# guanjq/targetdiff

Hardware: NVIDIA H100
Metric: molecules/sec (1000-step sampling, CrossDocked pocket shape) (higher is better)
Workload: dtype f32 (storage, LayerNorm, softmax, accumulation); GEMM operands as 2-piece bf16 splits on wgmma (3 products, ~16-bit operand mantissa)

## Files before the change

### targetdiff_b200/csrc/edge_mlp_v4.cu

```cuda
#include <stdio.h>
#include <stdlib.h>
#include <string.h>

#include "tdiff_common.cuh"
#include "hopper_mma.cuh"

namespace v4 {

constexpr int kTile = 64;
constexpr int kTabClassBytes = 2 * 128 * 128;
constexpr int kSrcStride = 512 + 32, kDst = 8;
constexpr int sSrc = 0, sDstRows = sSrc + kTile * kSrcStride, sMeta = sDstRows + kDst * 512, kStage = sMeta + kTile * 16;
constexpr int kMAtom = 32 * 128, kMPiece = 2 * kMAtom, kMImg = 2 * kMPiece;
template <int NOUT, bool FOLD>
struct Map {
  static constexpr int kCons = (NOUT == 128 && !FOLD) ? 3 : 2;
  static constexpr int kThreads = (kCons + 1) * 128;
  static constexpr int kProdRegs = kCons == 3 ? 32 : 40, kConsRegs = kCons == 3 ? 160 : 232;
  static constexpr int W = 0, T = W + 4 * 128 * 128, Par = T + kTabClassBytes, X = Par + 2 * 128 * 4,
                       M = X + kCons * 4 * 2 * 128 * 4, C = M + (FOLD ? kCons * kMImg : 0), Stage = C + (FOLD ? kCons * 32 * 4 : 0),
                       Bar = Stage + kCons * kStage, Smem = Bar + 8 * (1 + 2 * kCons);
  static constexpr bool kOrdered = kCons == 2;
  static constexpr int kPairBar = 1, kOrderBar = kPairBar + 2 * kCons, kFoldBar = kOrderBar + kCons;
  static_assert(M % 1024 == 0 && Stage % 128 == 0 && kStage % 128 == 0 && Smem <= 227 * 1024, "shared-memory map");
  static_assert(128 * kProdRegs + kCons * 128 * kConsRegs == kThreads * (65536 / kThreads / 8 * 8), "register split");
  static_assert(kFoldBar + kCons <= 16, "named barriers");
};

__device__ __forceinline__ uint32_t smem_u32(const void* p) { return (uint32_t)__cvta_generic_to_shared(p); }
__device__ __forceinline__ void mbar_init(uint32_t bar, uint32_t count) {
  asm volatile("mbarrier.init.shared::cta.b64 [%0], %1;" ::"r"(bar), "r"(count) : "memory");
}
__device__ __forceinline__ void mbar_wait(uint32_t bar, uint32_t parity) {
  asm volatile(
      "{\n\t.reg .pred p;\n\tWAIT_LOOP:\n\tmbarrier.try_wait.parity.shared::cta.b64 p, [%0], %1;\n\t@p bra WAIT_DONE;\n\tbra WAIT_LOOP;\n\t"
      "WAIT_DONE:\n\t}" ::"r"(bar), "r"(parity) : "memory");
}
__device__ __forceinline__ void mbar_expect_tx(uint32_t bar, uint32_t bytes) {
  asm volatile("mbarrier.arrive.expect_tx.shared::cta.b64 _, [%0], %1;" ::"r"(bar), "r"(bytes) : "memory");
}
__device__ __forceinline__ void bulk_g2s(uint32_t smem_dst, const void* gsrc, uint32_t bytes, uint32_t bar) {
  asm volatile("cp.async.bulk.shared::cluster.global.mbarrier::complete_tx::bytes [%0], [%1], %2, [%3];" ::"r"(smem_dst), "l"(gsrc), "r"(bytes),
               "r"(bar) : "memory");
}
__device__ __forceinline__ void fence_barrier_init() { asm volatile("fence.mbarrier_init.release.cluster;" ::: "memory"); }
__device__ __forceinline__ void mbar_arrive(uint32_t bar) { asm volatile("mbarrier.arrive.shared::cta.b64 _, [%0];" ::"r"(bar) : "memory"); }
__device__ __forceinline__ void mbar_expect_tx_only(uint32_t bar, uint32_t bytes) {
  asm volatile("mbarrier.expect_tx.shared::cta.b64 [%0], %1;" ::"r"(bar), "r"(bytes) : "memory");
}
__device__ __forceinline__ void named_bar_sync(int id, int nthreads) { asm volatile("bar.sync %0, %1;" ::"r"(id), "r"(nthreads) : "memory"); }
__device__ __forceinline__ void named_bar_arrive(int id, int nthreads) { asm volatile("bar.arrive %0, %1;" ::"r"(id), "r"(nthreads) : "memory"); }
template <int N> __device__ __forceinline__ void setmaxnreg_inc() { asm volatile("setmaxnreg.inc.sync.aligned.u32 %0;" ::"n"(N)); }
template <int N> __device__ __forceinline__ void setmaxnreg_dec() { asm volatile("setmaxnreg.dec.sync.aligned.u32 %0;" ::"n"(N)); }

__device__ __forceinline__ uint32_t cvt_bf16x2(float hi, float lo) {
  uint32_t d;
  asm("cvt.rn.bf16x2.f32 %0, %1, %2;" : "=r"(d) : "f"(hi), "f"(lo));
  return d;
}
__device__ __forceinline__ float ex2_approx(float x) { float y; asm("ex2.approx.ftz.f32 %0, %1;" : "=f"(y) : "f"(x)); return y; }
__device__ __forceinline__ void stg64(float* p, float a, float b) { asm volatile("st.global.v2.f32 [%0], {%1,%2};" ::"l"(p), "f"(a), "f"(b) : "memory"); }
__device__ __forceinline__ void stg128(float* p, float a, float b, float c, float d) {
  asm volatile("st.global.v4.f32 [%0], {%1,%2,%3,%4};" ::"l"(p), "f"(a), "f"(b), "f"(c), "f"(d) : "memory");
}

struct LnParams { float b[128]; float b2[128]; float mu[20]; };
struct AggArgs {
  const float* logits;
  const float* e_w;
  float* h;
  int key_softmax;
};

template <int N, int M, int LO_BIT>
__device__ __forceinline__ void transpose_reduce(float (&t)[N], int lane) {
  if constexpr (N > M) {
    constexpr int h = (N / M / 2) << LO_BIT;
    const bool up = lane & h;
#pragma unroll
    for (int i = 0; i < N / 2; ++i) {
      const float send = up ? t[i] : t[i + N / 2];
      const float keep = up ? t[i + N / 2] : t[i];
      t[i] = keep + __shfl_xor_sync(0xffffffffu, send, h);
    }
    transpose_reduce<N / 2, M, LO_BIT>(reinterpret_cast<float(&)[N / 2]>(t), lane);
  }
}
__device__ __forceinline__ void split2(float y0, float y1, uint32_t& hi, uint32_t& lo) {
  hi = cvt_bf16x2(y1, y0);
  const float r0 = __fsub_rn(y0, __uint_as_float(hi << 16)), r1 = __fsub_rn(y1, __uint_as_float(hi & 0xffff0000u));
  lo = cvt_bf16x2(r1, r0);
}

}

using namespace v4;

template <int NOUT, bool FOLD>
__global__ void __launch_bounds__(Map<NOUT, FOLD>::kThreads, 1)
edge_mlp_v4_kernel(const float* __restrict__ P, int zero_row, const int* __restrict__ src, const unsigned char* __restrict__ etype,
                   const float* __restrict__ dist_arr, const int* __restrict__ row_nodes, long long n_dst, long long split_dst,
                   const int* __restrict__ d_counts, int k, int offA, int offB, const unsigned char* __restrict__ w2_image,
                   const unsigned char* __restrict__ tab_image, float coeff, const float* __restrict__ qnode, float* __restrict__ out, int out_by_slot, AggArgs agg,
                   int cls, const __grid_constant__ LnParams lp) {
  static_assert(!FOLD || NOUT == 128, "the fold applies to the key MLPs");
  using L = Map<NOUT, FOLD>;
  constexpr int kCons = L::kCons, kThreads = L::kThreads;
  extern __shared__ __align__(1024) unsigned char smem_raw[];
  const uint32_t sbase = smem_u32(smem_raw);
  const uint32_t sW = sbase + L::W, sT = sbase + L::T, sBar = sbase + L::Bar;
  float* const s_b = reinterpret_cast<float*>(smem_raw + L::Par);
  float* const s_b2 = s_b + 128;
  const int tid = threadIdx.x, lane = tid & 31, warp = __shfl_sync(0xffffffffu, tid >> 5, 0);
  const int w = warp & 3, q = lane & 3;
  const int kshift = (k & (k - 1)) == 0 ? __ffs(k) - 1 : -1;
  auto row_dst = [&](long long idx, int& j) -> unsigned {
    const unsigned a = kshift >= 0 ? (unsigned)idx >> kshift : (unsigned)idx / (unsigned)k;
    j = (int)((unsigned)idx - a * (unsigned)k);
    return a;
  };

  if ((sbase & 1023u) != 0) __trap();
  if (d_counts) { n_dst = d_counts[0]; split_dst = d_counts[1]; }
  const long long n_rows = n_dst * k, split_rows = split_dst * k;
  const long long row_lo = cls ? split_rows : 0, row_hi = cls ? n_rows : split_rows;
  const long long n_tiles = row_hi > row_lo ? (row_hi - row_lo + kTile - 1) / kTile : 0;
  const long long my_tiles = (n_tiles > blockIdx.x) ? (n_tiles - blockIdx.x + gridDim.x - 1) / gridDim.x : 0;
  auto full_bar = [&](int c) { return sBar + 8u * (1 + c); };
  auto empty_bar = [&](int c) { return sBar + 8u * (1 + kCons + c); };

  constexpr int kWAtom = NOUT * 128;
  constexpr int kWPiece = 2 * kWAtom;
  constexpr uint32_t kWBytes = FOLD ? 4u * 128 * 128 : 2u * kWPiece;
  if (tid == 0) {
    mbar_init(sBar, 1);
    for (int c = 0; c < kCons; ++c) { mbar_init(full_bar(c), 32); mbar_init(empty_bar(c), 128); }
    fence_barrier_init();
    mbar_expect_tx(sBar, kWBytes + kTabClassBytes);
    bulk_g2s(sW, w2_image, kWBytes, sBar);
    bulk_g2s(sT, tab_image + (size_t)cls * kTabClassBytes, kTabClassBytes, sBar);
  }
  for (int i = tid; i < 128; i += kThreads) { s_b[i] = lp.b[i]; s_b2[i] = lp.b2[i]; }
  __syncthreads();

  if (warp < 4) {
    setmaxnreg_dec<L::kProdRegs>();
    if (warp >= kCons) return;
    const int c = warp;
    const uint32_t st = sbase + L::Stage + (uint32_t)c * kStage;
    for (long long it = c, use = 0; it < my_tiles; it += kCons, ++use) {
      const long long tile = blockIdx.x + it * (long long)gridDim.x, row0 = row_lo + tile * kTile;
      int j0;
      const unsigned a0 = row_dst(row0, j0);
      const long long last = (row0 + kTile - 1 < row_hi ? row0 + kTile - 1 : row_hi - 1);
      const int n_d = min(kDst, (int)(row_dst(last, j0) - a0) + 1);
      int s[2];
      int4 meta[2];
#pragma unroll
      for (int h = 0; h < 2; ++h) {
        const long long idx = row0 + lane + 32 * h;
        int jj = 0, ty = 3, slot = 0, node = -1;
        float dist = 0.f;
        s[h] = -1;
        if (idx < n_rows) {
          const unsigned a = row_dst(idx, jj);
          slot = a - a0 < (unsigned)kDst ? (int)(a - a0) + 1 : 0;
          node = row_nodes[a];
          if (node >= 0) {
            const size_t e = (size_t)node * k + jj;
            s[h] = src[e]; ty = etype[e]; dist = dist_arr[e];
          }
        }
        meta[h] = make_int4(node, s[h], __float_as_int(dist), ty | (slot << 8) | (jj << 16));
      }
      int dnode = -1;
      if (lane < n_d) dnode = row_nodes[a0 + lane];
      mbar_wait(empty_bar(c), (uint32_t)(use & 1) ^ 1u);
#pragma unroll
      for (int h = 0; h < 2; ++h) *reinterpret_cast<int4*>(smem_raw + L::Stage + c * kStage + sMeta + 16 * (lane + 32 * h)) = meta[h];
      if (lane == 0) mbar_expect_tx_only(full_bar(c), (uint32_t)(kTile + (FOLD ? 2 : 1) * n_d) * 512u);
      __syncwarp();
#pragma unroll
      for (int h = 0; h < 2; ++h)
        bulk_g2s(st + sSrc + (uint32_t)(lane + 32 * h) * kSrcStride, P + (size_t)(s[h] >= 0 ? s[h] : zero_row) * TD_NPROJ + offB, 512u, full_bar(c));
      if (lane < n_d) bulk_g2s(st + sDstRows + (uint32_t)lane * 512u, P + (size_t)(dnode >= 0 ? dnode : zero_row) * TD_NPROJ + offA, 512u, full_bar(c));
      if (FOLD && lane < n_d) bulk_g2s(st + sDstRows + (uint32_t)(2 + lane) * 512u, qnode + (size_t)(dnode >= 0 ? dnode : 0) * TD_H, 512u, full_bar(c));
      mbar_arrive(full_bar(c));
    }
    return;
  }

  setmaxnreg_inc<L::kConsRegs>();
  const int cwg = (warp >> 2) - 1;
  float mu[5];
#pragma unroll
  for (int m = 0; m < 5; ++m) mu[m] = lp.mu[5 * q + m];
  const float coeff2 = coeff * 1.4426950408889634f;
  mbar_wait(sBar, 0);

  const int r_base = 16 * w + (lane >> 2);
  const int pair_bar = L::kPairBar + 2 * cwg + (w >> 1);
  float* const xslot = reinterpret_cast<float*>(smem_raw + L::X) + (size_t)(cwg * 4 + w) * 256;
  float* const xpart = xslot + ((w & 1) ? -256 : 256);
  const bool do_agg = !FOLD && NOUT == 128 && qnode == nullptr && agg.logits != nullptr;
  const bool key_sm = NOUT == 128 && qnode != nullptr && agg.key_softmax;
  const unsigned char* const stage = smem_raw + L::Stage + cwg * kStage;
  const int ct = tid & 127, fu = ct & 7, fg = ct >> 3;
  const int fhd = 8 * (fg & 1) + 4 * (fu >> 2) + (fu & 3), fs = fu >> 2, frun = (fg >> 1) ^ (((fu >> 1) & 1) << 2);
  const int fn0 = 16 * ((fhd >> 1) & 1) + 2 * (fhd >> 2) + (fhd & 1);
  unsigned char* const mimg = smem_raw + L::M + cwg * kMImg;
  float* const s_c = reinterpret_cast<float*>(smem_raw + L::C) + cwg * 32;
  const int srow = k == 32 ? (w >> 1) : 0;
  const int order_mine = L::kOrderBar + cwg, order_next = L::kOrderBar + (cwg + 1) % kCons;
  auto order_wait = [&] { if constexpr (L::kOrdered) named_bar_sync(order_mine, 256); };
  auto order_pass = [&] { if constexpr (L::kOrdered) named_bar_arrive(order_next, 256); };
  const long long n_iter = (my_tiles + kCons - 1) / kCons;
  if (n_iter == 0) return;
  if (cwg == kCons - 1) order_pass();
  int set = 0;

  for (long long n = 0; n < n_iter; ++n, set ^= 1) {
    const long long it = n * kCons + cwg;
    if (it >= my_tiles) {
      if constexpr (L::kOrdered)
        for (int phase = 0; phase < 2; ++phase) { order_wait(); order_pass(); }
      continue;
    }
    const long long row0 = row_lo + (blockIdx.x + it * (long long)gridDim.x) * kTile;
    long long idx[2];
    int node[2], s[2], ty[2], jj[2], dsl[2];
    float dist[2];
    mbar_wait(full_bar(cwg), (uint32_t)(n & 1));
#pragma unroll
    for (int h = 0; h < 2; ++h) {
      idx[h] = row0 + r_base + 8 * h;
      const int4 m4 = *reinterpret_cast<const int4*>(stage + sMeta + 16 * (r_base + 8 * h));
      node[h] = m4.x; s[h] = m4.y; dist[h] = __int_as_float(m4.z);
      ty[h] = m4.w & 0xff; dsl[h] = ((m4.w >> 8) & 0xff) - 1; jj[h] = m4.w >> 16;
    }
    float ewp[2] = {0.f, 0.f};
    float4 qf[2][2];
    if constexpr (FOLD) {
#pragma unroll
      for (int h = 0; h < 2; ++h)
        if (key_sm && idx[h] < n_rows && node[h] >= 0) ewp[h] = agg.e_w[(size_t)node[h] * k + jj[h]];
#pragma unroll
      for (int sl = 0; sl < 2; ++sl)
#pragma unroll
        for (int hf = 0; hf < 2; ++hf) {
          float4 v = make_float4(0.f, 0.f, 0.f, 0.f);
          if (sl == 0 || k == 32) {
            v = *reinterpret_cast<const float4*>(stage + sDstRows + (2 + sl) * 512 + 32 * fhd + 16 * (hf ^ fs));
            v.x *= 0.35355339059327373f; v.y *= 0.35355339059327373f; v.z *= 0.35355339059327373f; v.w *= 0.35355339059327373f;
          }
          qf[sl][hf] = v;
        }
    }
    uint32_t ghi[4][4], glo[4][4];
#pragma unroll
    for (int h = 0; h < 2; ++h) {
      const bool ok = s[h] >= 0;
      float v[8];
#pragma unroll
      for (int m = 0; m < 5; ++m) {
        const float t = dist[h] - mu[m];
        v[m] = ok ? ex2_approx(coeff2 * (t * t)) : 0.0f;
      }
      v[5] = (ok && q == 3) ? 1.0f : 0.0f;
      v[6] = v[7] = 0.0f;
      const int half = ty[h] < 2 ? 1 : 0;
#pragma unroll
      for (int kk = 0; kk < 4; ++kk)
#pragma unroll
        for (int hk = 0; hk < 2; ++hk) {
          uint32_t hi, lo;
          split2(v[4 * (kk & 1) + 2 * hk], v[4 * (kk & 1) + 2 * hk + 1], hi, lo);
          const bool own = (kk >> 1) == half;
          ghi[kk][h + 2 * hk] = own ? hi : 0u;
          glo[kk][h + 2 * hk] = own ? lo : 0u;
        }
    }
    float x[64];
#pragma unroll
    for (int h = 0; h < 2; ++h) {
      const bool valid = s[h] >= 0;
      const float* ps = reinterpret_cast<const float*>(stage + sSrc + (r_base + 8 * h) * kSrcStride) + 2 * q;
      const float* pd = (dsl[h] >= 0 ? reinterpret_cast<const float*>(stage + sDstRows + dsl[h] * 512)
                                     : P + (size_t)(valid ? node[h] : zero_row) * TD_NPROJ + offA) + 2 * q;
#pragma unroll
      for (int i = 0; i < 16; ++i) {
        const float2 b = *reinterpret_cast<const float2*>(ps + 8 * i);
        float2 a = make_float2(0.f, 0.f);
        if (valid) a = *reinterpret_cast<const float2*>(pd + 8 * i);
        x[4 * i + 2 * h] = __fadd_rn(b.x, a.x);
        x[4 * i + 2 * h + 1] = __fadd_rn(b.y, a.y);
      }
    }
    mbar_arrive(empty_bar(cwg));
    wgmma_fence();
    order_wait();
#pragma unroll
    for (int term = 0; term < 3; ++term) {
#pragma unroll
      for (int kk = 0; kk < 4; ++kk)
        wgmma_n128_rs(x, term == 2 ? glo[kk] : ghi[kk], gmma_desc_sw128(sT + (term == 1 ? kTabClassBytes / 2 : 0) + kk * 32),
                      1u);
    }
    wgmma_commit();
    order_pass();
    if constexpr (FOLD) {
      const float* const w2s = reinterpret_cast<const float*>(smem_raw + L::W) + 8 * fhd;
#pragma unroll
      for (int jr = 0; jr < 2; ++jr) {
        const int f0 = 64 * jr + 8 * frun;
        float mv[2][8];
#pragma unroll
        for (int jf = 0; jf < 8; ++jf) {
          const float4 wa = *reinterpret_cast<const float4*>(w2s + (f0 + jf) * 128 + 4 * fs);
          const float4 wb = *reinterpret_cast<const float4*>(w2s + (f0 + jf) * 128 + 4 * (fs ^ 1));
#pragma unroll
          for (int sl = 0; sl < 2; ++sl) {
            const float4 qa = qf[sl][0], qb = qf[sl][1];
            const float pa = __fmaf_rn(wa.w, qa.w, __fmaf_rn(wa.z, qa.z, __fmaf_rn(wa.y, qa.y, wa.x * qa.x)));
            const float pb = __fmaf_rn(wb.w, qb.w, __fmaf_rn(wb.z, qb.z, __fmaf_rn(wb.y, qb.y, wb.x * qb.x)));
            mv[sl][jf] = pa + pb;
          }
        }
#pragma unroll
        for (int sl = 0; sl < 2; ++sl) {
          uint4 hi, lo;
          split2(mv[sl][0], mv[sl][1], hi.x, lo.x);
          split2(mv[sl][2], mv[sl][3], hi.y, lo.y);
          split2(mv[sl][4], mv[sl][5], hi.z, lo.z);
          split2(mv[sl][6], mv[sl][7], hi.w, lo.w);
          const int nr = fn0 + 8 * sl;
          const int off = jr * kMAtom + (nr >> 3) * 1024 + (nr & 7) * 128 + ((frun ^ (nr & 7)) << 4);
          *reinterpret_cast<uint4*>(mimg + off) = hi;
          *reinterpret_cast<uint4*>(mimg + kMPiece + off) = lo;
        }
      }
      if (fg < 2)
#pragma unroll
        for (int sl = 0; sl < 2; ++sl) {
          const float4 ba = *reinterpret_cast<const float4*>(s_b2 + 8 * fhd + 4 * fs), bb = *reinterpret_cast<const float4*>(s_b2 + 8 * fhd + 4 * (fs ^ 1));
          const float4 qa = qf[sl][0], qb = qf[sl][1];
          const float pa = __fmaf_rn(ba.w, qa.w, __fmaf_rn(ba.z, qa.z, __fmaf_rn(ba.y, qa.y, ba.x * qa.x)));
          const float pb = __fmaf_rn(bb.w, qb.w, __fmaf_rn(bb.z, qb.z, __fmaf_rn(bb.y, qb.y, bb.x * qb.x)));
          s_c[16 * sl + fhd] = pa + pb;
        }
      asm volatile("fence.proxy.async.shared::cta;" ::: "memory");
    }
    wgmma_wait_all();
    float rstd[2];
#pragma unroll
    for (int h = 0; h < 2; ++h) {
      float qa = 0.f, qb = 0.f;
#pragma unroll
      for (int i = 0; i < 16; ++i) {
        qa = __fmaf_rn(x[4 * i + 2 * h], x[4 * i + 2 * h], qa);
        qb = __fmaf_rn(x[4 * i + 2 * h + 1], x[4 * i + 2 * h + 1], qb);
      }
      float var = qa + qb;
      var += __shfl_xor_sync(0xffffffffu, var, 1);
      var += __shfl_xor_sync(0xffffffffu, var, 2);
      rstd[h] = rsqrtf(var * (1.0f / 128.0f) + 1e-5f);
    }
    uint32_t ahi[8][4], alo[8][4];
#pragma unroll
    for (int kk = 0; kk < 8; ++kk)
#pragma unroll
      for (int r = 0; r < 4; ++r) {
        const int h = r & 1, col = 16 * kk + 8 * (r >> 1) + 2 * q, e = 8 * kk + 2 * r;
        const float2 b = *reinterpret_cast<const float2*>(s_b + col);
        const float y0 = __fmaf_rn(x[e], rstd[h], b.x), y1 = __fmaf_rn(x[e + 1], rstd[h], b.y);
        split2(fmaxf(y0, 0.f), fmaxf(y1, 0.f), ahi[kk][r], alo[kk][r]);
      }
    float o[NOUT / 2];
    if constexpr (FOLD) {
      named_bar_sync(L::kFoldBar + cwg, 128);
#pragma unroll
      for (int sl = 0; sl < 2; ++sl) {
        const float4 cv = *reinterpret_cast<const float4*>(s_c + 16 * sl + 4 * q);
#pragma unroll
        for (int h = 0; h < 2; ++h) {
          o[4 * sl + 2 * h] = cv.x; o[4 * sl + 2 * h + 1] = cv.y;
          o[4 * (2 + sl) + 2 * h] = cv.z; o[4 * (2 + sl) + 2 * h + 1] = cv.w;
        }
      }
    }
    wgmma_fence();
    order_wait();
#pragma unroll
    for (int term = 0; term < 3; ++term) {
#pragma unroll
      for (int kk = 0; kk < 8; ++kk) {
        if constexpr (FOLD) {
          const uint64_t desc = gmma_desc_sw128(sbase + L::M + cwg * kMImg + (term == 1 ? kMPiece : 0) + (kk >> 2) * kMAtom + (kk & 3) * 32);
          wgmma_n32_rs(reinterpret_cast<float(&)[16]>(o), term == 2 ? alo[kk] : ahi[kk], desc, 1u);
        } else {
          const uint64_t desc = gmma_desc_sw128(sW + (term == 1 ? kWPiece : 0) + (kk >> 2) * kWAtom + (kk & 3) * 32);
          if constexpr (NOUT == 128) wgmma_n128_rs(o, term == 2 ? alo[kk] : ahi[kk], desc, (term | kk) ? 1u : 0u);
          else wgmma_n16_rs(o, term == 2 ? alo[kk] : ahi[kk], desc, (term | kk) ? 1u : 0u);
        }
      }
    }
    wgmma_commit();
    order_pass();
    wgmma_wait_all();

    long long orow[2];
    bool owrite[2];
#pragma unroll
    for (int h = 0; h < 2; ++h) {
      orow[h] = out_by_slot ? ((long long)node[h] * k + jj[h]) : idx[h];
      owrite[h] = idx[h] < n_rows && node[h] >= 0;
    }
    if constexpr (NOUT == 16) {
#pragma unroll
      for (int h = 0; h < 2; ++h)
        if (owrite[h])
#pragma unroll
          for (int i = 0; i < 2; ++i) {
            const float2 bb = *reinterpret_cast<const float2*>(s_b2 + 8 * i + 2 * q);
            stg64(out + (size_t)orow[h] * 16 + 8 * i + 2 * q, o[4 * i + 2 * h] + bb.x, o[4 * i + 2 * h + 1] + bb.y);
          }
    } else if (do_agg) {
      const int dnode = node[0];
      const bool active = dnode >= 0;
      const int ccol = 64 * (w & 1) + 2 * lane;
      float2 hin = make_float2(0.f, 0.f);
      if (active) hin = *reinterpret_cast<const float2*>(agg.h + (size_t)dnode * TD_H + ccol);
      float wt[2][16];
#pragma unroll
      for (int h = 0; h < 2; ++h)
#pragma unroll
        for (int i = 0; i < 4; ++i) {
          float4 t4 = make_float4(0.f, 0.f, 0.f, 0.f);
          if (active) t4 = __ldg(reinterpret_cast<const float4*>(agg.logits + (size_t)idx[h] * TD_HEADS + 4 * i));
          wt[h][4 * i] = t4.x; wt[h][4 * i + 1] = t4.y; wt[h][4 * i + 2] = t4.z; wt[h][4 * i + 3] = t4.w;
        }
      float t[32];
#pragma unroll
      for (int i = 0; i < 16; ++i) {
        const float2 bb = *reinterpret_cast<const float2*>(s_b2 + 8 * i + 2 * q);
#pragma unroll
        for (int c = 0; c < 2; ++c) {
          const float b = c ? bb.y : bb.x;
          t[2 * i + c] = __fadd_rn(__fmul_rn(__fadd_rn(o[4 * i + c], b), wt[0][i]), __fmul_rn(__fadd_rn(o[4 * i + 2 + c], b), wt[1][i]));
        }
      }
      transpose_reduce<32, 4, 2>(t, lane);
      float* slot = xslot + 128 * set;
      const int c0 = 16 * (lane >> 2) + 2 * q;
      *reinterpret_cast<float2*>(slot + c0) = make_float2(t[0], t[1]);
      *reinterpret_cast<float2*>(slot + c0 + 8) = make_float2(t[2], t[3]);
      named_bar_sync(pair_bar, 64);
      if (active) {
        const float* se = ((w & 1) ? xpart : xslot) + 128 * set;
        const float* so = ((w & 1) ? xslot : xpart) + 128 * set;
        const float2 a = *reinterpret_cast<const float2*>(se + ccol), b = *reinterpret_cast<const float2*>(so + ccol);
        *reinterpret_cast<float2*>(agg.h + (size_t)dnode * TD_H + ccol) = make_float2(hin.x + (a.x + b.x), hin.y + (a.y + b.y));
      }
    } else if (!FOLD && qnode == nullptr) {
#pragma unroll
      for (int h = 0; h < 2; ++h)
        if (owrite[h])
#pragma unroll
          for (int i = 0; i < 16; ++i) {
            const float2 bb = *reinterpret_cast<const float2*>(s_b2 + 8 * i + 2 * q);
            stg64(out + (size_t)orow[h] * 128 + 8 * i + 2 * q, o[4 * i + 2 * h] + bb.x, o[4 * i + 2 * h + 1] + bb.y);
          }
    } else {
      float lg[32];
      if constexpr (FOLD) {
#pragma unroll
        for (int h = 0; h < 2; ++h)
#pragma unroll
          for (int u = 0; u < 4; ++u) {
            const int e0 = 4 * (2 * (u >> 1)) + 2 * h + (u & 1);
            lg[4 * h + u] = srow ? o[e0 + 4] : o[e0];
          }
      } else {
#pragma unroll
        for (int h = 0; h < 2; ++h) {
          const float* qrow = qnode + (size_t)(node[h] >= 0 ? node[h] : 0) * TD_H + 2 * q;
#pragma unroll
          for (int i = 0; i < 16; ++i) {
            const float2 qv = __ldg(reinterpret_cast<const float2*>(qrow + 8 * i));
            const float2 bb = *reinterpret_cast<const float2*>(s_b2 + 8 * i + 2 * q);
            lg[8 * (i >> 2) + 4 * h + (i & 3)] = __fmaf_rn(o[4 * i + 2 * h + 1] + bb.y, qv.y, (o[4 * i + 2 * h] + bb.x) * qv.x);
          }
        }
        transpose_reduce<32, 8, 0>(lg, lane);
#pragma unroll
        for (int u = 0; u < 8; ++u) lg[u] *= 0.35355339059327373f;
      }
      if (key_sm) {
        bool valid_e[2];
        float ew[2];
#pragma unroll
        for (int h = 0; h < 2; ++h) {
          valid_e[h] = false; ew[h] = 0.f;
          if (owrite[h]) {
            valid_e[h] = s[h] >= 0;
            ew[h] = FOLD ? ewp[h] : agg.e_w[(size_t)node[h] * k + jj[h]];
          }
        }
        float mx[4], sm[4];
#pragma unroll
        for (int u = 0; u < 4; ++u) {
          lg[u] = valid_e[0] ? lg[u] * 1.4426950408889634f : -INFINITY;
          lg[4 + u] = valid_e[1] ? lg[4 + u] * 1.4426950408889634f : -INFINITY;
          mx[u] = fmaxf(lg[u], lg[4 + u]);
#pragma unroll
          for (int m = 4; m < 32; m <<= 1) mx[u] = fmaxf(mx[u], __shfl_xor_sync(0xffffffffu, mx[u], m));
        }
        if (lane < 4) *reinterpret_cast<float4*>(xslot + 4 * q) = make_float4(mx[0], mx[1], mx[2], mx[3]);
        named_bar_sync(pair_bar, 64);
        const float4 pm = *reinterpret_cast<const float4*>(xpart + 4 * q);
        mx[0] = fmaxf(mx[0], pm.x); mx[1] = fmaxf(mx[1], pm.y); mx[2] = fmaxf(mx[2], pm.z); mx[3] = fmaxf(mx[3], pm.w);
#pragma unroll
        for (int u = 0; u < 4; ++u) {
          lg[u] = valid_e[0] ? ex2_approx(lg[u] - mx[u]) : 0.0f;
          lg[4 + u] = valid_e[1] ? ex2_approx(lg[4 + u] - mx[u]) : 0.0f;
          sm[u] = lg[u] + lg[4 + u];
#pragma unroll
          for (int m = 4; m < 32; m <<= 1) sm[u] += __shfl_xor_sync(0xffffffffu, sm[u], m);
        }
        if (lane < 4) *reinterpret_cast<float4*>(xslot + 128 + 4 * q) = make_float4(sm[0], sm[1], sm[2], sm[3]);
        named_bar_sync(pair_bar, 64);
        const float4 ps = *reinterpret_cast<const float4*>(xpart + 128 + 4 * q);
        const float pl[4] = {ps.x, ps.y, ps.z, ps.w};
#pragma unroll
        for (int u = 0; u < 4; ++u) {
          const float l = sm[u] + pl[u];
          const float inv = l > 0.0f ? 1.0f / l : 0.0f;
          lg[u] = lg[u] * ew[0] * inv;
          lg[4 + u] = lg[4 + u] * ew[1] * inv;
        }
#pragma unroll
        for (int h = 0; h < 2; ++h)
          if (idx[h] < n_rows) stg128(out + (size_t)idx[h] * TD_HEADS + 4 * q, lg[4 * h], lg[4 * h + 1], lg[4 * h + 2], lg[4 * h + 3]);
      } else {
#pragma unroll
        for (int h = 0; h < 2; ++h)
          if (owrite[h]) stg128(out + (size_t)orow[h] * TD_HEADS + 4 * q, lg[4 * h], lg[4 * h + 1], lg[4 * h + 2], lg[4 * h + 3]);
      }
    }
  }
  if (cwg == 0) order_wait();
}

void td_launch_edge_mlp_v4(const float* P, int zero_row, const int* src, const unsigned char* etype, const float* dist, const int* row_nodes, long long n_dst,
                           long long split_dst, const int* d_counts, int k, const TdMlp& m, const float* h_offsets, float coeff,
                           const float* h_ln_b, const float* h_b2, const float* qnode, float* out, int out_by_slot,
                           const float* agg_logits, const float* agg_e_w, float* agg_h, int key_softmax, int sm_count, cudaStream_t st) {
  if (n_dst == 0) return;
  LnParams lp;
  memcpy(lp.b, h_ln_b, sizeof(lp.b));
  memset(lp.b2, 0, sizeof(lp.b2));
  memcpy(lp.b2, h_b2, sizeof(float) * (size_t)m.nout);
  memcpy(lp.mu, h_offsets, sizeof(lp.mu));
  static size_t opted128[TD_MAX_DEVICES] = {0}, opted16[TD_MAX_DEVICES] = {0}, optedF[TD_MAX_DEVICES] = {0};
  td_opt_in_smem(edge_mlp_v4_kernel<128, false>, Map<128, false>::Smem, opted128);
  td_opt_in_smem(edge_mlp_v4_kernel<16, false>, Map<16, false>::Smem, opted16);
  td_opt_in_smem(edge_mlp_v4_kernel<128, true>, Map<128, true>::Smem, optedF);
  AggArgs agg = {agg_logits, agg_e_w, agg_h, (key_softmax && k == 32) ? 1 : 0};
  const bool fold = m.nout == 128 && qnode && (k == 32 || k == 64);
  const long long n_cls[2] = {split_dst, n_dst - split_dst};
  for (int cls = 0; cls < 2; ++cls) {
    if (n_cls[cls] == 0) continue;
    const long long n_tiles = (n_cls[cls] * k + kTile - 1) / kTile;
    const int grid = (int)(n_tiles < sm_count ? n_tiles : sm_count);
    if (m.nout == 16)
      edge_mlp_v4_kernel<16, false><<<grid, Map<16, false>::kThreads, Map<16, false>::Smem, st>>>(
          P, zero_row, src, etype, dist, row_nodes, n_dst, split_dst, d_counts, k, m.offA, m.offB, m.w2_img, m.tabcls_img, coeff, nullptr,
          out, out_by_slot, agg, cls, lp);
    else if (fold)
      edge_mlp_v4_kernel<128, true><<<grid, Map<128, true>::kThreads, Map<128, true>::Smem, st>>>(
          P, zero_row, src, etype, dist, row_nodes, n_dst, split_dst, d_counts, k, m.offA, m.offB,
          reinterpret_cast<const unsigned char*>(m.w2t), m.tabcls_img, coeff, qnode, out, out_by_slot, agg, cls, lp);
    else
      edge_mlp_v4_kernel<128, false><<<grid, Map<128, false>::kThreads, Map<128, false>::Smem, st>>>(
          P, zero_row, src, etype, dist, row_nodes, n_dst, split_dst, d_counts, k, m.offA, m.offB, m.w2_img, m.tabcls_img, coeff, qnode,
          out, out_by_slot, agg, cls, lp);
  }
}
```

### targetdiff_b200/csrc/hopper_mma.cuh

```cuda
#pragma once
#include <stdint.h>

__device__ __forceinline__ uint64_t gmma_desc_sw128(uint32_t smem_addr) {
  return (uint64_t)((smem_addr >> 4) & 0x3FFF) | ((uint64_t)1 << 16) | ((uint64_t)(1024 >> 4) << 32) | ((uint64_t)1 << 62);
}
__device__ __forceinline__ void wgmma_fence() { asm volatile("wgmma.fence.sync.aligned;" ::: "memory"); }
__device__ __forceinline__ void wgmma_commit() { asm volatile("wgmma.commit_group.sync.aligned;" ::: "memory"); }
__device__ __forceinline__ void wgmma_wait_all() { asm volatile("wgmma.wait_group.sync.aligned 0;" ::: "memory"); }

__device__ __forceinline__ void wgmma_n128(float (&d)[64], uint64_t desc_a, uint64_t desc_b, uint32_t accumulate) {
  asm volatile(
      "{\n\t.reg .pred p;\n\tsetp.ne.b32 p, %66, 0;\n\t"
      "wgmma.mma_async.sync.aligned.m64n128k16.f32.bf16.bf16 {%0,%1,%2,%3,%4,%5,%6,%7,%8,%9,%10,%11,%12,%13,%14,%15,%16,%17,%18,%19,%20,%21,%22,%23,%24,%25,%26,%27,%28,%29,%30,%31,%32,%33,%34,%35,%36,%37,%38,%39,%40,%41,%42,%43,%44,%45,%46,%47,%48,%49,%50,%51,%52,%53,%54,%55,%56,%57,%58,%59,%60,%61,%62,%63}, %64, %65, p, 1, 1, 0, 0;\n\t}"
      : "+f"(d[0]), "+f"(d[1]), "+f"(d[2]), "+f"(d[3]), "+f"(d[4]), "+f"(d[5]), "+f"(d[6]), "+f"(d[7]), "+f"(d[8]), "+f"(d[9]), "+f"(d[10]), "+f"(d[11]), "+f"(d[12]), "+f"(d[13]), "+f"(d[14]), "+f"(d[15]), "+f"(d[16]), "+f"(d[17]), "+f"(d[18]), "+f"(d[19]), "+f"(d[20]), "+f"(d[21]), "+f"(d[22]), "+f"(d[23]), "+f"(d[24]), "+f"(d[25]), "+f"(d[26]), "+f"(d[27]), "+f"(d[28]), "+f"(d[29]), "+f"(d[30]), "+f"(d[31]), "+f"(d[32]), "+f"(d[33]), "+f"(d[34]), "+f"(d[35]), "+f"(d[36]), "+f"(d[37]), "+f"(d[38]), "+f"(d[39]), "+f"(d[40]), "+f"(d[41]), "+f"(d[42]), "+f"(d[43]), "+f"(d[44]), "+f"(d[45]), "+f"(d[46]), "+f"(d[47]), "+f"(d[48]), "+f"(d[49]), "+f"(d[50]), "+f"(d[51]), "+f"(d[52]), "+f"(d[53]), "+f"(d[54]), "+f"(d[55]), "+f"(d[56]), "+f"(d[57]), "+f"(d[58]), "+f"(d[59]), "+f"(d[60]), "+f"(d[61]), "+f"(d[62]), "+f"(d[63])
      : "l"(desc_a), "l"(desc_b), "r"(accumulate) : "memory");
}

__device__ __forceinline__ void wgmma_n128_rs(float (&d)[64], const uint32_t (&a)[4], uint64_t desc_b, uint32_t accumulate) {
  asm volatile(
      "{\n\t.reg .pred p;\n\tsetp.ne.b32 p, %69, 0;\n\t"
      "wgmma.mma_async.sync.aligned.m64n128k16.f32.bf16.bf16 {%0,%1,%2,%3,%4,%5,%6,%7,%8,%9,%10,%11,%12,%13,%14,%15,%16,%17,%18,%19,%20,%21,%22,%23,%24,%25,%26,%27,%28,%29,%30,%31,%32,%33,%34,%35,%36,%37,%38,%39,%40,%41,%42,%43,%44,%45,%46,%47,%48,%49,%50,%51,%52,%53,%54,%55,%56,%57,%58,%59,%60,%61,%62,%63}, {%64,%65,%66,%67}, %68, p, 1, 1, 0;\n\t}"
      : "+f"(d[0]), "+f"(d[1]), "+f"(d[2]), "+f"(d[3]), "+f"(d[4]), "+f"(d[5]), "+f"(d[6]), "+f"(d[7]), "+f"(d[8]), "+f"(d[9]), "+f"(d[10]), "+f"(d[11]), "+f"(d[12]), "+f"(d[13]), "+f"(d[14]), "+f"(d[15]), "+f"(d[16]), "+f"(d[17]), "+f"(d[18]), "+f"(d[19]), "+f"(d[20]), "+f"(d[21]), "+f"(d[22]), "+f"(d[23]), "+f"(d[24]), "+f"(d[25]), "+f"(d[26]), "+f"(d[27]), "+f"(d[28]), "+f"(d[29]), "+f"(d[30]), "+f"(d[31]), "+f"(d[32]), "+f"(d[33]), "+f"(d[34]), "+f"(d[35]), "+f"(d[36]), "+f"(d[37]), "+f"(d[38]), "+f"(d[39]), "+f"(d[40]), "+f"(d[41]), "+f"(d[42]), "+f"(d[43]), "+f"(d[44]), "+f"(d[45]), "+f"(d[46]), "+f"(d[47]), "+f"(d[48]), "+f"(d[49]), "+f"(d[50]), "+f"(d[51]), "+f"(d[52]), "+f"(d[53]), "+f"(d[54]), "+f"(d[55]), "+f"(d[56]), "+f"(d[57]), "+f"(d[58]), "+f"(d[59]), "+f"(d[60]), "+f"(d[61]), "+f"(d[62]), "+f"(d[63])
      : "r"(a[0]), "r"(a[1]), "r"(a[2]), "r"(a[3]), "l"(desc_b), "r"(accumulate) : "memory");
}

__device__ __forceinline__ void wgmma_n32_rs(float (&d)[16], const uint32_t (&a)[4], uint64_t desc_b, uint32_t accumulate) {
  asm volatile(
      "{\n\t.reg .pred p;\n\tsetp.ne.b32 p, %21, 0;\n\t"
      "wgmma.mma_async.sync.aligned.m64n32k16.f32.bf16.bf16 {%0,%1,%2,%3,%4,%5,%6,%7,%8,%9,%10,%11,%12,%13,%14,%15}, {%16,%17,%18,%19}, %20, p, 1, 1, 0;\n\t}"
      : "+f"(d[0]), "+f"(d[1]), "+f"(d[2]), "+f"(d[3]), "+f"(d[4]), "+f"(d[5]), "+f"(d[6]), "+f"(d[7]), "+f"(d[8]), "+f"(d[9]), "+f"(d[10]), "+f"(d[11]),
        "+f"(d[12]), "+f"(d[13]), "+f"(d[14]), "+f"(d[15])
      : "r"(a[0]), "r"(a[1]), "r"(a[2]), "r"(a[3]), "l"(desc_b), "r"(accumulate) : "memory");
}

__device__ __forceinline__ void wgmma_n16_rs(float (&d)[8], const uint32_t (&a)[4], uint64_t desc_b, uint32_t accumulate) {
  asm volatile(
      "{\n\t.reg .pred p;\n\tsetp.ne.b32 p, %13, 0;\n\t"
      "wgmma.mma_async.sync.aligned.m64n16k16.f32.bf16.bf16 {%0,%1,%2,%3,%4,%5,%6,%7}, {%8,%9,%10,%11}, %12, p, 1, 1, 0;\n\t}"
      : "+f"(d[0]), "+f"(d[1]), "+f"(d[2]), "+f"(d[3]), "+f"(d[4]), "+f"(d[5]), "+f"(d[6]), "+f"(d[7])
      : "r"(a[0]), "r"(a[1]), "r"(a[2]), "r"(a[3]), "l"(desc_b), "r"(accumulate) : "memory");
}
```

Baseline: 19.00.

## Drop folded query path; add L2 prefetch of query/aggregate rows and ordered-issue removal

Removes the FOLD variant, which folded the query vector into the second-layer weights per tile and used a 2-consumer ordered wgmma schedule. Key MLPs now always use the plain 3-consumer N=128 path and compute the logits as a dot product with qnode rows read from global memory; when both rows share a node, one load is reused. The producer warps issue bulk L2 prefetches of the destination node's query/h row and e_w row ahead of consumption. This trades the per-tile fold GEMM and its ordering barriers for a larger second GEMM and extra global loads of the query rows.

After: 19.20, median of 6. 1.1% higher.

```diff
diff --git a/targetdiff_b200/csrc/edge_mlp_v4.cu b/targetdiff_b200/csrc/edge_mlp_v4.cu
--- a/targetdiff_b200/csrc/edge_mlp_v4.cu
+++ b/targetdiff_b200/csrc/edge_mlp_v4.cu
@@ -11,20 +11,18 @@
 constexpr int kTabClassBytes = 2 * 128 * 128;
 constexpr int kSrcStride = 512 + 32, kDst = 8;
 constexpr int sSrc = 0, sDstRows = sSrc + kTile * kSrcStride, sMeta = sDstRows + kDst * 512, kStage = sMeta + kTile * 16;
-constexpr int kMAtom = 32 * 128, kMPiece = 2 * kMAtom, kMImg = 2 * kMPiece;
-template <int NOUT, bool FOLD>
+template <int NOUT>
 struct Map {
-  static constexpr int kCons = (NOUT == 128 && !FOLD) ? 3 : 2;
+  static constexpr int kCons = 3;
   static constexpr int kThreads = (kCons + 1) * 128;
-  static constexpr int kProdRegs = kCons == 3 ? 32 : 40, kConsRegs = kCons == 3 ? 160 : 232;
+  static constexpr int kProdRegs = 32, kConsRegs = 160;
   static constexpr int W = 0, T = W + 4 * 128 * 128, Par = T + kTabClassBytes, X = Par + 2 * 128 * 4,
-                       M = X + kCons * 4 * 2 * 128 * 4, C = M + (FOLD ? kCons * kMImg : 0), Stage = C + (FOLD ? kCons * 32 * 4 : 0),
+                       Stage = X + kCons * 4 * 2 * 128 * 4,
                        Bar = Stage + kCons * kStage, Smem = Bar + 8 * (1 + 2 * kCons);
-  static constexpr bool kOrdered = kCons == 2;
-  static constexpr int kPairBar = 1, kOrderBar = kPairBar + 2 * kCons, kFoldBar = kOrderBar + kCons;
-  static_assert(M % 1024 == 0 && Stage % 128 == 0 && kStage % 128 == 0 && Smem <= 227 * 1024, "shared-memory map");
+  static constexpr int kPairBar = 1;
+  static_assert(T % 1024 == 0 && Stage % 128 == 0 && kStage % 128 == 0 && Smem <= 227 * 1024, "shared-memory map");
   static_assert(128 * kProdRegs + kCons * 128 * kConsRegs == kThreads * (65536 / kThreads / 8 * 8), "register split");
-  static_assert(kFoldBar + kCons <= 16, "named barriers");
+  static_assert(kPairBar + 2 * kCons <= 16, "named barriers");
 };
 
 __device__ __forceinline__ uint32_t smem_u32(const void* p) { return (uint32_t)__cvta_generic_to_shared(p); }
@@ -42,6 +40,9 @@
 __device__ __forceinline__ void bulk_g2s(uint32_t smem_dst, const void* gsrc, uint32_t bytes, uint32_t bar) {
   asm volatile("cp.async.bulk.shared::cluster.global.mbarrier::complete_tx::bytes [%0], [%1], %2, [%3];" ::"r"(smem_dst), "l"(gsrc), "r"(bytes),
                "r"(bar) : "memory");
+}
+__device__ __forceinline__ void bulk_prefetch_l2(const void* gsrc, uint32_t bytes) {
+  asm volatile("cp.async.bulk.prefetch.L2.global [%0], %1;" ::"l"(gsrc), "r"(bytes) : "memory");
 }
 __device__ __forceinline__ void fence_barrier_init() { asm volatile("fence.mbarrier_init.release.cluster;" ::: "memory"); }
 __device__ __forceinline__ void mbar_arrive(uint32_t bar) { asm volatile("mbarrier.arrive.shared::cta.b64 _, [%0];" ::"r"(bar) : "memory"); }
@@ -96,15 +97,14 @@
 
 using namespace v4;
 
-template <int NOUT, bool FOLD>
-__global__ void __launch_bounds__(Map<NOUT, FOLD>::kThreads, 1)
+template <int NOUT>
+__global__ void __launch_bounds__(Map<NOUT>::kThreads, 1)
 edge_mlp_v4_kernel(const float* __restrict__ P, int zero_row, const int* __restrict__ src, const unsigned char* __restrict__ etype,
                    const float* __restrict__ dist_arr, const int* __restrict__ row_nodes, long long n_dst, long long split_dst,
                    const int* __restrict__ d_counts, int k, int offA, int offB, const unsigned char* __restrict__ w2_image,
                    const unsigned char* __restrict__ tab_image, float coeff, const float* __restrict__ qnode, float* __restrict__ out, int out_by_slot, AggArgs agg,
                    int cls, const __grid_constant__ LnParams lp) {
-  static_assert(!FOLD || NOUT == 128, "the fold applies to the key MLPs");
-  using L = Map<NOUT, FOLD>;
+  using L = Map<NOUT>;
   constexpr int kCons = L::kCons, kThreads = L::kThreads;
   extern __shared__ __align__(1024) unsigned char smem_raw[];
   const uint32_t sbase = smem_u32(smem_raw);
@@ -131,7 +131,7 @@
 
   constexpr int kWAtom = NOUT * 128;
   constexpr int kWPiece = 2 * kWAtom;
-  constexpr uint32_t kWBytes = FOLD ? 4u * 128 * 128 : 2u * kWPiece;
+  constexpr uint32_t kWBytes = 2u * kWPiece;
   if (tid == 0) {
     mbar_init(sBar, 1);
     for (int c = 0; c < kCons; ++c) { mbar_init(full_bar(c), 32); mbar_init(empty_bar(c), 128); }
@@ -142,10 +142,13 @@
   }
   for (int i = tid; i < 128; i += kThreads) { s_b[i] = lp.b[i]; s_b2[i] = lp.b2[i]; }
   __syncthreads();
+  const bool do_agg = NOUT == 128 && qnode == nullptr && agg.logits != nullptr;
+  const bool key_sm = NOUT == 128 && qnode != nullptr && agg.key_softmax;
 
   if (warp < 4) {
     setmaxnreg_dec<L::kProdRegs>();
     if (warp >= kCons) return;
+    const float* const pf_dst = NOUT != 128 ? nullptr : qnode ? qnode : do_agg ? agg.h : nullptr;
     const int c = warp;
     const uint32_t st = sbase + L::Stage + (uint32_t)c * kStage;
     for (long long it = c, use = 0; it < my_tiles; it += kCons, ++use) {
@@ -175,16 +178,19 @@
       }
       int dnode = -1;
       if (lane < n_d) dnode = row_nodes[a0 + lane];
+      if (pf_dst && dnode >= 0) {
+        bulk_prefetch_l2(pf_dst + (size_t)dnode * TD_H, TD_H * 4u);
+        if (key_sm) bulk_prefetch_l2(agg.e_w + (size_t)dnode * k, (uint32_t)k * 4u);
+      }
       mbar_wait(empty_bar(c), (uint32_t)(use & 1) ^ 1u);
 #pragma unroll
       for (int h = 0; h < 2; ++h) *reinterpret_cast<int4*>(smem_raw + L::Stage + c * kStage + sMeta + 16 * (lane + 32 * h)) = meta[h];
-      if (lane == 0) mbar_expect_tx_only(full_bar(c), (uint32_t)(kTile + (FOLD ? 2 : 1) * n_d) * 512u);
+      if (lane == 0) mbar_expect_tx_only(full_bar(c), (uint32_t)(kTile + n_d) * 512u);
       __syncwarp();
 #pragma unroll
       for (int h = 0; h < 2; ++h)
         bulk_g2s(st + sSrc + (uint32_t)(lane + 32 * h) * kSrcStride, P + (size_t)(s[h] >= 0 ? s[h] : zero_row) * TD_NPROJ + offB, 512u, full_bar(c));
       if (lane < n_d) bulk_g2s(st + sDstRows + (uint32_t)lane * 512u, P + (size_t)(dnode >= 0 ? dnode : zero_row) * TD_NPROJ + offA, 512u, full_bar(c));
-      if (FOLD && lane < n_d) bulk_g2s(st + sDstRows + (uint32_t)(2 + lane) * 512u, qnode + (size_t)(dnode >= 0 ? dnode : 0) * TD_H, 512u, full_bar(c));
       mbar_arrive(full_bar(c));
     }
     return;
@@ -202,30 +208,9 @@
   const int pair_bar = L::kPairBar + 2 * cwg + (w >> 1);
   float* const xslot = reinterpret_cast<float*>(smem_raw + L::X) + (size_t)(cwg * 4 + w) * 256;
   float* const xpart = xslot + ((w & 1) ? -256 : 256);
-  const bool do_agg = !FOLD && NOUT == 128 && qnode == nullptr && agg.logits != nullptr;
-  const bool key_sm = NOUT == 128 && qnode != nullptr && agg.key_softmax;
   const unsigned char* const stage = smem_raw + L::Stage + cwg * kStage;
-  const int ct = tid & 127, fu = ct & 7, fg = ct >> 3;
-  const int fhd = 8 * (fg & 1) + 4 * (fu >> 2) + (fu & 3), fs = fu >> 2, frun = (fg >> 1) ^ (((fu >> 1) & 1) << 2);
-  const int fn0 = 16 * ((fhd >> 1) & 1) + 2 * (fhd >> 2) + (fhd & 1);
-  unsigned char* const mimg = smem_raw + L::M + cwg * kMImg;
-  float* const s_c = reinterpret_cast<float*>(smem_raw + L::C) + cwg * 32;
-  const int srow = k == 32 ? (w >> 1) : 0;
-  const int order_mine = L::kOrderBar + cwg, order_next = L::kOrderBar + (cwg + 1) % kCons;
-  auto order_wait = [&] { if constexpr (L::kOrdered) named_bar_sync(order_mine, 256); };
-  auto order_pass = [&] { if constexpr (L::kOrdered) named_bar_arrive(order_next, 256); };
-  const long long n_iter = (my_tiles + kCons - 1) / kCons;
-  if (n_iter == 0) return;
-  if (cwg == kCons - 1) order_pass();
   int set = 0;
-
-  for (long long n = 0; n < n_iter; ++n, set ^= 1) {
-    const long long it = n * kCons + cwg;
-    if (it >= my_tiles) {
-      if constexpr (L::kOrdered)
-        for (int phase = 0; phase < 2; ++phase) { order_wait(); order_pass(); }
-      continue;
-    }
+  for (long long n = 0, it = cwg; it < my_tiles; ++n, it += kCons, set ^= 1) {
     const long long row0 = row_lo + (blockIdx.x + it * (long long)gridDim.x) * kTile;
     long long idx[2];
     int node[2], s[2], ty[2], jj[2], dsl[2];
@@ -237,24 +222,6 @@
       const int4 m4 = *reinterpret_cast<const int4*>(stage + sMeta + 16 * (r_base + 8 * h));
       node[h] = m4.x; s[h] = m4.y; dist[h] = __int_as_float(m4.z);
       ty[h] = m4.w & 0xff; dsl[h] = ((m4.w >> 8) & 0xff) - 1; jj[h] = m4.w >> 16;
-    }
-    float ewp[2] = {0.f, 0.f};
-    float4 qf[2][2];
-    if constexpr (FOLD) {
-#pragma unroll
-      for (int h = 0; h < 2; ++h)
-        if (key_sm && idx[h] < n_rows && node[h] >= 0) ewp[h] = agg.e_w[(size_t)node[h] * k + jj[h]];
-#pragma unroll
-      for (int sl = 0; sl < 2; ++sl)
-#pragma unroll
-        for (int hf = 0; hf < 2; ++hf) {
-          float4 v = make_float4(0.f, 0.f, 0.f, 0.f);
-          if (sl == 0 || k == 32) {
-            v = *reinterpret_cast<const float4*>(stage + sDstRows + (2 + sl) * 512 + 32 * fhd + 16 * (hf ^ fs));
-            v.x *= 0.35355339059327373f; v.y *= 0.35355339059327373f; v.z *= 0.35355339059327373f; v.w *= 0.35355339059327373f;
-          }
-          qf[sl][hf] = v;
-        }
     }
     uint32_t ghi[4][4], glo[4][4];
 #pragma unroll
@@ -298,7 +265,6 @@
     }
     mbar_arrive(empty_bar(cwg));
     wgmma_fence();
-    order_wait();
 #pragma unroll
     for (int term = 0; term < 3; ++term) {
 #pragma unroll
@@ -307,49 +273,6 @@
                       1u);
     }
     wgmma_commit();
-    order_pass();
-    if constexpr (FOLD) {
-      const float* const w2s = reinterpret_cast<const float*>(smem_raw + L::W) + 8 * fhd;
-#pragma unroll
-      for (int jr = 0; jr < 2; ++jr) {
-        const int f0 = 64 * jr + 8 * frun;
-        float mv[2][8];
-#pragma unroll
-        for (int jf = 0; jf < 8; ++jf) {
-          const float4 wa = *reinterpret_cast<const float4*>(w2s + (f0 + jf) * 128 + 4 * fs);
-          const float4 wb = *reinterpret_cast<const float4*>(w2s + (f0 + jf) * 128 + 4 * (fs ^ 1));
-#pragma unroll
-          for (int sl = 0; sl < 2; ++sl) {
-            const float4 qa = qf[sl][0], qb = qf[sl][1];
-            const float pa = __fmaf_rn(wa.w, qa.w, __fmaf_rn(wa.z, qa.z, __fmaf_rn(wa.y, qa.y, wa.x * qa.x)));
-            const float pb = __fmaf_rn(wb.w, qb.w, __fmaf_rn(wb.z, qb.z, __fmaf_rn(wb.y, qb.y, wb.x * qb.x)));
-            mv[sl][jf] = pa + pb;
-          }
-        }
-#pragma unroll
-        for (int sl = 0; sl < 2; ++sl) {
-          uint4 hi, lo;
-          split2(mv[sl][0], mv[sl][1], hi.x, lo.x);
-          split2(mv[sl][2], mv[sl][3], hi.y, lo.y);
-          split2(mv[sl][4], mv[sl][5], hi.z, lo.z);
-          split2(mv[sl][6], mv[sl][7], hi.w, lo.w);
-          const int nr = fn0 + 8 * sl;
-          const int off = jr * kMAtom + (nr >> 3) * 1024 + (nr & 7) * 128 + ((frun ^ (nr & 7)) << 4);
-          *reinterpret_cast<uint4*>(mimg + off) = hi;
-          *reinterpret_cast<uint4*>(mimg + kMPiece + off) = lo;
-        }
-      }
-      if (fg < 2)
-#pragma unroll
-        for (int sl = 0; sl < 2; ++sl) {
-          const float4 ba = *reinterpret_cast<const float4*>(s_b2 + 8 * fhd + 4 * fs), bb = *reinterpret_cast<const float4*>(s_b2 + 8 * fhd + 4 * (fs ^ 1));
-          const float4 qa = qf[sl][0], qb = qf[sl][1];
-          const float pa = __fmaf_rn(ba.w, qa.w, __fmaf_rn(ba.z, qa.z, __fmaf_rn(ba.y, qa.y, ba.x * qa.x)));
-          const float pb = __fmaf_rn(bb.w, qb.w, __fmaf_rn(bb.z, qb.z, __fmaf_rn(bb.y, qb.y, bb.x * qb.x)));
-          s_c[16 * sl + fhd] = pa + pb;
-        }
-      asm volatile("fence.proxy.async.shared::cta;" ::: "memory");
-    }
     wgmma_wait_all();
     float rstd[2];
 #pragma unroll
@@ -376,36 +299,17 @@
         split2(fmaxf(y0, 0.f), fmaxf(y1, 0.f), ahi[kk][r], alo[kk][r]);
       }
     float o[NOUT / 2];
-    if constexpr (FOLD) {
-      named_bar_sync(L::kFoldBar + cwg, 128);
-#pragma unroll
-      for (int sl = 0; sl < 2; ++sl) {
-        const float4 cv = *reinterpret_cast<const float4*>(s_c + 16 * sl + 4 * q);
-#pragma unroll
-        for (int h = 0; h < 2; ++h) {
-          o[4 * sl + 2 * h] = cv.x; o[4 * sl + 2 * h + 1] = cv.y;
-          o[4 * (2 + sl) + 2 * h] = cv.z; o[4 * (2 + sl) + 2 * h + 1] = cv.w;
-        }
-      }
-    }
     wgmma_fence();
-    order_wait();
 #pragma unroll
     for (int term = 0; term < 3; ++term) {
 #pragma unroll
       for (int kk = 0; kk < 8; ++kk) {
-        if constexpr (FOLD) {
-          const uint64_t desc = gmma_desc_sw128(sbase + L::M + cwg * kMImg + (term == 1 ? kMPiece : 0) + (kk >> 2) * kMAtom + (kk & 3) * 32);
-          wgmma_n32_rs(reinterpret_cast<float(&)[16]>(o), term == 2 ? alo[kk] : ahi[kk], desc, 1u);
-        } else {
-          const uint64_t desc = gmma_desc_sw128(sW + (term == 1 ? kWPiece : 0) + (kk >> 2) * kWAtom + (kk & 3) * 32);
-          if constexpr (NOUT == 128) wgmma_n128_rs(o, term == 2 ? alo[kk] : ahi[kk], desc, (term | kk) ? 1u : 0u);
-          else wgmma_n16_rs(o, term == 2 ? alo[kk] : ahi[kk], desc, (term | kk) ? 1u : 0u);
-        }
+        const uint64_t desc = gmma_desc_sw128(sW + (term == 1 ? kWPiece : 0) + (kk >> 2) * kWAtom + (kk & 3) * 32);
+        if constexpr (NOUT == 128) wgmma_n128_rs(o, term == 2 ? alo[kk] : ahi[kk], desc, (term | kk) ? 1u : 0u);
+        else wgmma_n16_rs(o, term == 2 ? alo[kk] : ahi[kk], desc, (term | kk) ? 1u : 0u);
       }
     }
     wgmma_commit();
-    order_pass();
     wgmma_wait_all();
 
     long long orow[2];
@@ -461,7 +365,7 @@
         const float2 a = *reinterpret_cast<const float2*>(se + ccol), b = *reinterpret_cast<const float2*>(so + ccol);
         *reinterpret_cast<float2*>(agg.h + (size_t)dnode * TD_H + ccol) = make_float2(hin.x + (a.x + b.x), hin.y + (a.y + b.y));
       }
-    } else if (!FOLD && qnode == nullptr) {
+    } else if (qnode == nullptr) {
 #pragma unroll
       for (int h = 0; h < 2; ++h)
         if (owrite[h])
@@ -472,29 +376,26 @@
           }
     } else {
       float lg[32];
-      if constexpr (FOLD) {
-#pragma unroll
-        for (int h = 0; h < 2; ++h)
-#pragma unroll
-          for (int u = 0; u < 4; ++u) {
-            const int e0 = 4 * (2 * (u >> 1)) + 2 * h + (u & 1);
-            lg[4 * h + u] = srow ? o[e0 + 4] : o[e0];
-          }
-      } else {
-#pragma unroll
-        for (int h = 0; h < 2; ++h) {
-          const float* qrow = qnode + (size_t)(node[h] >= 0 ? node[h] : 0) * TD_H + 2 * q;
-#pragma unroll
-          for (int i = 0; i < 16; ++i) {
-            const float2 qv = __ldg(reinterpret_cast<const float2*>(qrow + 8 * i));
-            const float2 bb = *reinterpret_cast<const float2*>(s_b2 + 8 * i + 2 * q);
-            lg[8 * (i >> 2) + 4 * h + (i & 3)] = __fmaf_rn(o[4 * i + 2 * h + 1] + bb.y, qv.y, (o[4 * i + 2 * h] + bb.x) * qv.x);
-          }
-        }
-        transpose_reduce<32, 8, 0>(lg, lane);
-#pragma unroll
-        for (int u = 0; u < 8; ++u) lg[u] *= 0.35355339059327373f;
-      }
+      float ewv[2] = {0.f, 0.f};
+#pragma unroll
+      for (int h = 0; h < 2; ++h)
+        if (key_sm && owrite[h]) ewv[h] = agg.e_w[(size_t)node[h] * k + jj[h]];
+      {
+        const float* q0 = qnode + (size_t)(node[0] >= 0 ? node[0] : 0) * TD_H + 2 * q;
+        const float* q1 = qnode + (size_t)(node[1] >= 0 ? node[1] : 0) * TD_H + 2 * q;
+        const bool same = node[0] == node[1];
+#pragma unroll
+        for (int i = 0; i < 16; ++i) {
+          const float2 qa = __ldg(reinterpret_cast<const float2*>(q0 + 8 * i));
+          const float2 qb = same ? qa : __ldg(reinterpret_cast<const float2*>(q1 + 8 * i));
+          const float2 bb = *reinterpret_cast<const float2*>(s_b2 + 8 * i + 2 * q);
+          lg[8 * (i >> 2) + (i & 3)] = __fmaf_rn(o[4 * i + 1] + bb.y, qa.y, (o[4 * i] + bb.x) * qa.x);
+          lg[8 * (i >> 2) + 4 + (i & 3)] = __fmaf_rn(o[4 * i + 3] + bb.y, qb.y, (o[4 * i + 2] + bb.x) * qb.x);
+        }
+      }
+      transpose_reduce<32, 8, 0>(lg, lane);
+#pragma unroll
+      for (int u = 0; u < 8; ++u) lg[u] *= 0.35355339059327373f;
       if (key_sm) {
         bool valid_e[2];
         float ew[2];
@@ -503,7 +404,7 @@
           valid_e[h] = false; ew[h] = 0.f;
           if (owrite[h]) {
             valid_e[h] = s[h] >= 0;
-            ew[h] = FOLD ? ewp[h] : agg.e_w[(size_t)node[h] * k + jj[h]];
+            ew[h] = ewv[h];
           }
         }
         float mx[4], sm[4];
@@ -548,7 +449,6 @@
       }
     }
   }
-  if (cwg == 0) order_wait();
 }
 
 void td_launch_edge_mlp_v4(const float* P, int zero_row, const int* src, const unsigned char* etype, const float* dist, const int* row_nodes, long long n_dst,
@@ -561,27 +461,21 @@
   memset(lp.b2, 0, sizeof(lp.b2));
   memcpy(lp.b2, h_b2, sizeof(float) * (size_t)m.nout);
   memcpy(lp.mu, h_offsets, sizeof(lp.mu));
-  static size_t opted128[TD_MAX_DEVICES] = {0}, opted16[TD_MAX_DEVICES] = {0}, optedF[TD_MAX_DEVICES] = {0};
-  td_opt_in_smem(edge_mlp_v4_kernel<128, false>, Map<128, false>::Smem, opted128);
-  td_opt_in_smem(edge_mlp_v4_kernel<16, false>, Map<16, false>::Smem, opted16);
-  td_opt_in_smem(edge_mlp_v4_kernel<128, true>, Map<128, true>::Smem, optedF);
+  static size_t opted128[TD_MAX_DEVICES] = {0}, opted16[TD_MAX_DEVICES] = {0};
+  td_opt_in_smem(edge_mlp_v4_kernel<128>, Map<128>::Smem, opted128);
+  td_opt_in_smem(edge_mlp_v4_kernel<16>, Map<16>::Smem, opted16);
   AggArgs agg = {agg_logits, agg_e_w, agg_h, (key_softmax && k == 32) ? 1 : 0};
-  const bool fold = m.nout == 128 && qnode && (k == 32 || k == 64);
   const long long n_cls[2] = {split_dst, n_dst - split_dst};
   for (int cls = 0; cls < 2; ++cls) {
     if (n_cls[cls] == 0) continue;
     const long long n_tiles = (n_cls[cls] * k + kTile - 1) / kTile;
     const int grid = (int)(n_tiles < sm_count ? n_tiles : sm_count);
     if (m.nout == 16)
-      edge_mlp_v4_kernel<16, false><<<grid, Map<16, false>::kThreads, Map<16, false>::Smem, st>>>(
+      edge_mlp_v4_kernel<16><<<grid, Map<16>::kThreads, Map<16>::Smem, st>>>(
           P, zero_row, src, etype, dist, row_nodes, n_dst, split_dst, d_counts, k, m.offA, m.offB, m.w2_img, m.tabcls_img, coeff, nullptr,
           out, out_by_slot, agg, cls, lp);
-    else if (fold)
-      edge_mlp_v4_kernel<128, true><<<grid, Map<128, true>::kThreads, Map<128, true>::Smem, st>>>(
-          P, zero_row, src, etype, dist, row_nodes, n_dst, split_dst, d_counts, k, m.offA, m.offB,
-          reinterpret_cast<const unsigned char*>(m.w2t), m.tabcls_img, coeff, qnode, out, out_by_slot, agg, cls, lp);
     else
-      edge_mlp_v4_kernel<128, false><<<grid, Map<128, false>::kThreads, Map<128, false>::Smem, st>>>(
+      edge_mlp_v4_kernel<128><<<grid, Map<128>::kThreads, Map<128>::Smem, st>>>(
           P, zero_row, src, etype, dist, row_nodes, n_dst, split_dst, d_counts, k, m.offA, m.offB, m.w2_img, m.tabcls_img, coeff, qnode,
           out, out_by_slot, agg, cls, lp);
   }
diff --git a/targetdiff_b200/csrc/hopper_mma.cuh b/targetdiff_b200/csrc/hopper_mma.cuh
--- a/targetdiff_b200/csrc/hopper_mma.cuh
+++ b/targetdiff_b200/csrc/hopper_mma.cuh
@@ -24,15 +24,6 @@
       : "r"(a[0]), "r"(a[1]), "r"(a[2]), "r"(a[3]), "l"(desc_b), "r"(accumulate) : "memory");
 }
 
-__device__ __forceinline__ void wgmma_n32_rs(float (&d)[16], const uint32_t (&a)[4], uint64_t desc_b, uint32_t accumulate) {
-  asm volatile(
-      "{\n\t.reg .pred p;\n\tsetp.ne.b32 p, %21, 0;\n\t"
-      "wgmma.mma_async.sync.aligned.m64n32k16.f32.bf16.bf16 {%0,%1,%2,%3,%4,%5,%6,%7,%8,%9,%10,%11,%12,%13,%14,%15}, {%16,%17,%18,%19}, %20, p, 1, 1, 0;\n\t}"
-      : "+f"(d[0]), "+f"(d[1]), "+f"(d[2]), "+f"(d[3]), "+f"(d[4]), "+f"(d[5]), "+f"(d[6]), "+f"(d[7]), "+f"(d[8]), "+f"(d[9]), "+f"(d[10]), "+f"(d[11]),
-        "+f"(d[12]), "+f"(d[13]), "+f"(d[14]), "+f"(d[15])
-      : "r"(a[0]), "r"(a[1]), "r"(a[2]), "r"(a[3]), "l"(desc_b), "r"(accumulate) : "memory");
-}
-
 __device__ __forceinline__ void wgmma_n16_rs(float (&d)[8], const uint32_t (&a)[4], uint64_t desc_b, uint32_t accumulate) {
   asm volatile(
       "{\n\t.reg .pred p;\n\tsetp.ne.b32 p, %13, 0;\n\t"
```
